# lesliegaga/GPT-SoVITS

Measured on AMD Instinct MI355X. Metric: synthesised audio sec/sec (1/RTF), v2 pipeline, higher is better.
Workload: dtype f16

## Files before the change

### gpt-sovits_amd/csrc/common.h

```cpp
#pragma once
#include <hip/hip_runtime.h>

#include <type_traits>
#include <hip/hip_fp16.h>
#include <stdint.h>
#include <stdio.h>
#include <stdarg.h>
#include <string.h>

#include "../../include/gsv.h"

namespace gsv {

typedef _Float16 h8 __attribute__((ext_vector_type(8)));
typedef _Float16 h4 __attribute__((ext_vector_type(4)));
typedef _Float16 h2 __attribute__((ext_vector_type(2)));
typedef float f4 __attribute__((ext_vector_type(4)));
typedef float f16v __attribute__((ext_vector_type(16)));

void set_error(const char* fmt, ...);

#define GSV_HIP(expr)                                                                   \
  do {                                                                                  \
    hipError_t _e = (expr);                                                             \
// ... 121 lines not shown
  float scale = 1.0f;
  int accumulate = 0;
  int out_f32 = 0;
  int res_f32 = 0;
  int ups_u = 0, ups_pad = 0, ups_cout = 0;
  int Z = 1;
  long long xz = 0, wz = 0, yz = 0, rz = 0;
  unsigned long long* prof = nullptr;
  int bz = 0;
  int xcd_order = 0;
  int w_nt = 0;
  int z_res = 0;
  const int* row_seg = nullptr;
};
enum { ROUTE_GEMM_SK = 1, ROUTE_GEMM_T64 = 2, ROUTE_CONV_WIDE = 3, ROUTE_GEMM_LDS = 4, ROUTE_CONV_LDS = 5, ROUTE_CONV_NARROW = 6,
       ROUTE_CONV_GEMM = 7, ROUTE_CONV_PAIR = 8 };
enum { ROUTE_RES = 1, ROUTE_ACCU = 2, ROUTE_ALLW = 4, ROUTE_WNT = 8, ROUTE_SEG = 16 };
constexpr unsigned long long route_code(int family, int dtype, int p0 = 0, int p1 = 0, int p2 = 0, int p3 = 0, int p4 = 0, int flags = 0) {
  return (unsigned long long)(family & 255) | (unsigned long long)(dtype & 255) << 8 | (unsigned long long)(p0 & 255) << 16 |
         (unsigned long long)(p1 & 255) << 24 | (unsigned long long)(p2 & 255) << 32 | (unsigned long long)(p3 & 255) << 40 |
         (unsigned long long)(p4 & 255) << 48 | (unsigned long long)(flags & 255) << 56;
}
constexpr int route_flags(bool res, bool accu, bool allw = false, bool wnt = false) {
  return (res ? ROUTE_RES : 0) | (accu ? ROUTE_ACCU : 0) | (allw ? ROUTE_ALLW : 0) | (wnt ? ROUTE_WNT : 0);
}
void set_conv_route(unsigned long long code);
int launch_seg_rows(int dtype, int out_f32, void* y, int ldy, int col0, int C, int rows, const int* row_seg, const float* tab, int ldb,
                    hipStream_t s);

int launch_conv_gemm(int dtype, const ConvArgs& a, hipStream_t s);

struct ConvPairArgs {
  const _Float16* x = nullptr;
  const _Float16* w1 = nullptr;
  const float* b1 = nullptr;
  const _Float16* w2 = nullptr;
  const float* b2 = nullptr;
  _Float16* y = nullptr;
  int T = 0, C = 0, taps = 0, dil = 1, ldx = 0, ldy = 0;
  float scale = 1.f;
  int accumulate = 0;
};
bool conv_pair_supported(int dtype, int C, int taps, int dil, int T, bool seg);
bool conv_pair_eligible(int dtype, int C, int taps, int dil, int T, bool seg);
int launch_conv_pair(const ConvPairArgs& a, hipStream_t s);
// ... 27 lines not shown
```

### gpt-sovits_amd/csrc/ops.hip

```cpp
#include "common.h"
#include "engine.h"

namespace gsv {

static thread_local char g_err[1024] = "";
void set_error(const char* fmt, ...) {
  va_list ap;
  va_start(ap, fmt);
  vsnprintf(g_err, sizeof(g_err), fmt, ap);
  va_end(ap);
}
const char* get_error() { return g_err; }

static thread_local unsigned long long g_conv_route = 0;
static thread_local unsigned long long g_pair_route = 0;
void set_conv_route(unsigned long long code) {
  g_conv_route = code;
  if ((code & 255) == ROUTE_CONV_PAIR) g_pair_route = code;
}

template <typename T> __global__ void convert_kernel(const float* __restrict__ s, T* __restrict__ d, long long n) {
  long long i = (long long)blockIdx.x * blockDim.x + threadIdx.x;
  long long stride = (long long)gridDim.x * blockDim.x;
  for (; i < n; i += stride) d[i] = (T)s[i];
// ... 318 lines not shown
  GSV_REQUIRE(word && pos && ids && pos_ids && gamma && beta && y && rows > 0 && n_word > 0 && n_pos > 0, "op_embed_ln: bad argument");
  GSV_REQUIRE(C >= 1 && C <= 1024, "op_embed_ln: C = %d, the row is held in registers up to 1024", C);
  hipLaunchKernelGGL(gsv::embed_ln_kernel, dim3(gsv::cdiv(rows, 4)), dim3(256), 0, (hipStream_t)stream, word, pos, add, ids, pos_ids,
                     gamma, beta, (_Float16*)y, rows, C, n_word, n_pos, eps);
  GSV_HIP(hipGetLastError());
  return GSV_OK;
}

int gsv_op_flash_rel96(const void* qkv, int T, int heads, float scale, const float* rel_k, const float* rel_v, void* vt_scratch,
                       void* out, gsv_stream_t stream) {
  const int H = heads * 96;
  return gsv::launch_flash_rel96_f16(qkv, 3 * H, (const _Float16*)qkv + H, 3 * H, (const _Float16*)qkv + 2 * H, 3 * H, vt_scratch, T, heads,
                                     scale, rel_k, rel_v, out, H, (hipStream_t)stream);
}

int gsv_op_conv1d(const gsv_conv_desc* d, int dtype, gsv_stream_t stream) {
  gsv::ConvArgs a;
  a.x = d->x; a.w = d->w; a.bias = d->bias; a.y = d->y; a.res = d->res; a.gate = d->gate;
  a.T_in = d->T_in; a.T_out = d->T_out; a.Cin = d->Cin; a.Cout = d->Cout; a.taps = d->taps;
  a.stride = d->stride; a.dil = d->dil; a.pad = d->pad;
  a.ldx = d->Cin; a.ldw = d->taps * d->Cin;
  a.pre_act = d->pre_act; a.pre_slope = d->pre_slope; a.post_act = d->post_act; a.scale = d->scale;
  a.accumulate = d->accumulate; a.out_f32 = d->out_f32;
  a.res_f32 = d->res_dtype == 0 ? d->out_f32 : d->res_dtype == 1;
  a.y_col0 = d->y_col0; a.w_nt = d->w_nt; a.z_res = d->z_res;
  if (d->ups_u > 0) {
    a.ups_u = d->ups_u; a.ups_pad = d->ups_pad; a.ups_cout = d->Cout / d->ups_u;
    a.ldy = a.ups_cout; a.ldr = a.ups_cout;
    a.T_virt = d->T_in + d->taps - 1;
  } else {
    a.ldy = d->Cout; a.ldr = d->Cout;
    a.T_virt = d->T_out;
  }
  if (d->ldx > 0) a.ldx = d->ldx;
  if (d->ldw > 0) a.ldw = d->ldw;
  if (d->ldy > 0) { a.ldy = d->ldy; a.ldr = d->ldy; }
  if (d->ldr > 0) a.ldr = d->ldr;
  if (d->Z > 1) { a.Z = d->Z; a.xz = d->xz; a.wz = d->wz; a.yz = d->yz; a.bz = d->bz; a.rz = d->rz ? d->rz : d->yz; }
  return gsv::launch_conv_gemm(dtype, a, (hipStream_t)stream);
}

int gsv_op_frame(const float* x, int n, int frame_len, int hop, int pad, int ld, int T_out, void* out, int dtype, gsv_stream_t stream) {
  GSV_REQUIRE(x && out && n > 0 && frame_len > 0 && hop > 0 && ld >= frame_len && T_out > 0, "op_frame: bad argument");
  GSV_REQUIRE(pad >= 0 && pad < n, "op_frame: reflect padding %d needs more than %d samples", pad, pad);
  GSV_REQUIRE((long long)(T_out - 1) * hop + frame_len - pad <= (long long)n + pad, "op_frame: frames run past the (padded) signal");
  GSV_REQUIRE(dtype == GSV_F16 || dtype == GSV_F32, "op_frame: bad dtype");
  hipStream_t s = (hipStream_t)stream;
  if (dtype == GSV_F16) hipLaunchKernelGGL(gsv::frame_kernel<_Float16>, dim3(T_out), dim3(256), 0, s, x, n, frame_len, hop, pad, ld, T_out, (_Float16*)out);
  else hipLaunchKernelGGL(gsv::frame_kernel<float>, dim3(T_out), dim3(256), 0, s, x, n, frame_len, hop, pad, ld, T_out, (float*)out);
  GSV_HIP(hipGetLastError());
  return GSV_OK;
}

int gsv_op_magnitude(const float* re_im, int T, int bins, float eps, int frame_ld, float* spec, gsv_stream_t stream) {
// ... 104 lines not shown
```

### gpt-sovits_amd/csrc/t2s.hip

```cpp
#include <math.h>
#include <string.h>
#include <stdlib.h>
#include <algorithm>
#include <string>
#include <vector>

#include "t2s_engine.h"

namespace gsv {

typedef float f4v __attribute__((ext_vector_type(4)));


enum { EPI_QKV = 0, EPI_RESID = 1, EPI_RELU = 2, EPI_LOGITS = 3 };

struct DecGemmArgs {
  const float* yin = nullptr;
  const float* gamma = nullptr;
  const float* beta = nullptr;
  float* xres_out = nullptr;
  const void* xin = nullptr;
  const void* w = nullptr;
  const float* bias = nullptr;
  int B = 0, K = 0, N = 0;
// ... 922 lines not shown
                   int32_t* out_tokens, int32_t* out_len, int* steps_run, gsv_stream_t stream) {
  GSV_REQUIRE(h && h->finalized && h->B > 0, "t2s_decode: call gsv_t2s_prefill first");
  struct Clear { gsv_t2s_t* h; ~Clear() { h->row_sampling_next.clear(); } } clear{h};
  GSV_REQUIRE(sp && out_tokens && out_len, "t2s_decode: null argument");
  GSV_REQUIRE(sp->max_steps >= 1, "t2s_decode: max_steps must be >= 1");
  GSV_REQUIRE(noise == nullptr || noise_rows == 1 || noise_rows == h->B, "t2s_decode: noise_rows must be 1 or B");
  return GSV_WITH_T(h, decode<T>(h, sp, noise, noise_rows, out_tokens, out_len, steps_run, (hipStream_t)stream));
}

int gsv_t2s_set_mega(gsv_t2s_t* h, int on) {
  GSV_REQUIRE(h, "t2s_set_mega: null handle");
  h->mega_on = on != 0;
  return GSV_OK;
}

int gsv_t2s_set_debug(gsv_t2s_t* h, const int32_t* force_tokens, float* logits_dump, int32_t* drawn_dump) {
  GSV_REQUIRE(h && h->finalized, "t2s_set_debug: handle not finalized");
  h->dbg_force = force_tokens; h->dbg_dump = logits_dump; h->dbg_drawn = drawn_dump;
  return GSV_OK;
}

int gsv_t2s_debug_stall(gsv_t2s_t* h, int member) {
  GSV_REQUIRE(h && h->finalized && member >= 0 && member < 32, "t2s_debug_stall: bad argument");
  h->dbg_stall = member + 1;
  return GSV_OK;
}

int gsv_t2s_engine_stats(gsv_t2s_t* h, int* engine_available, int* fallbacks, unsigned* last_error3) {
  GSV_REQUIRE(h && h->finalized, "t2s_engine_stats: handle not finalized");
  if (engine_available) *engine_available = h->mega.ready && h->mega.census != 0 ? 1 : 0;
// ... 101 lines not shown
```

### gpt-sovits_amd/csrc/t2s_engine.h

```cpp
#pragma once
#include "engine.h"
#include "t2s_sample.h"
#include "t2s_mega.h"

struct LayerW {
  void *qkv_w = nullptr, *out_w = nullptr, *w1 = nullptr, *w2 = nullptr;
  float *qkv_b = nullptr, *out_b = nullptr, *b1 = nullptr, *b2 = nullptr;
  float *n1w = nullptr, *n1b = nullptr, *n2w = nullptr, *n2b = nullptr;
};

struct gsv_t2s : gsveng::Ctx {
  gsv_t2s() : Ctx("t2s") {}
  gsv_t2s_config cfg;
  int max_batch, max_seq;
  std::vector<LayerW> layers;
  void* bert_w = nullptr; float* bert_b = nullptr;
  float *e_text = nullptr, *e_audio = nullptr, *pe = nullptr;
  void* pred_w = nullptr;
  float alpha_t = 1.f, alpha_a = 1.f;
  int pe_rows = 0;
  void* kv = nullptr; size_t kv_layer_stride = 0;
  int *d_x_len = nullptr, *d_row_off = nullptr, *d_ph_off = nullptr, *d_kv_len = nullptr, *d_active = nullptr,
      *d_step = nullptr, *d_n_active = nullptr, *d_ytok = nullptr;
  int ycap = 0;
// ... 7 lines not shown
  int* h_pinned = nullptr;
  gsv::StepParams* d_sp = nullptr;
  float *ybuf = nullptr, *xres = nullptr, *logits = nullptr;
  void *qbuf = nullptr, *abuf = nullptr, *hbuf = nullptr;
  size_t pf_rows = 0;
  void *pf_x = nullptr, *pf_qkv = nullptr, *pf_attn = nullptr, *pf_h = nullptr;
  void* pf_vt = nullptr; size_t pf_vt_cap = 0;
  float *pf_y = nullptr, *pf_bert = nullptr;
  void* pf_bert_t = nullptr;
  int B = 0, P = 0;
  int max_kv0 = 0;
  gsv::MegaState mega;
  hipEvent_t mega_ev[2] = {nullptr, nullptr};
  float last_decode_ms = 0.f; int last_decode_steps = 0; int last_decode_mode = 0;
  bool mega_on = true;
  const int* dbg_force = nullptr; float* dbg_dump = nullptr; int* dbg_drawn = nullptr; int dbg_stall = 0;
  std::map<int, hipGraphExec_t> graphs;
};

inline void* kv_ptr(gsv_t2s* h, int layer, int which) {
  return (char*)h->kv + ((size_t)(layer * 2 + which) * h->kv_layer_stride) * gsveng::esz(h);
}
```

### gpt-sovits_amd/csrc/t2s_prefill.hip

```cpp
#include <stdlib.h>
#include <type_traits>
#include <vector>

#include "t2s_engine.h"

namespace gsv {

template <typename T>
__global__ void embed_prefill_kernel(const int* __restrict__ phones, const int* __restrict__ prompts,
                                     const int* __restrict__ row_off, const int* __restrict__ ph_off,
                                     const int* __restrict__ x_len, const float* __restrict__ e_text,
                                     const float* __restrict__ e_audio, const float* __restrict__ bertp,
                                     const float* __restrict__ bert_bias, const float* __restrict__ pe, float alpha_t,
                                     float alpha_a, const int* __restrict__ plen, const int* __restrict__ poff, int d,
                                     T* __restrict__ x) {
  const int b = blockIdx.y;
  const int i = blockIdx.x;
  const int X = x_len[b], P = plen[b];
  if (i >= X + P) return;
  T* out = x + (long long)(row_off[b] + i) * d;
  if (i < X) {
    const int id = phones[ph_off[b] + i];
    const float* e = e_text + (long long)id * d;
    const float* bp = bertp ? bertp + (long long)(ph_off[b] + i) * d : nullptr;
// ... 250 lines not shown
  GSV_RC(dalloc(h, (void**)&h->pf_y, rows * d * 4));
  GSV_RC(dalloc(h, (void**)&h->pf_bert, rows * d * 4));
  GSV_RC(dalloc(h, &h->pf_bert_t, rows * (size_t)h->cfg.bert_dim * es));
  h->pf_rows = rows;
  return GSV_OK;
}

ConvArgs linear(const void* x, const void* w, const float* bias, void* y, int rows, int K, int N) {
  ConvArgs g;
  g.x = x; g.w = w; g.bias = bias; g.y = y;
  g.T_in = rows; g.T_out = rows; g.T_virt = rows; g.Cin = K; g.Cout = N; g.ldx = K; g.ldw = K; g.ldy = N;
  return g;
}

bool scalar_prefill_attn() { static const bool v = getenv("GSV_SCALAR_PREFILL_ATTN") != nullptr; return v; }
bool prefill_split_scatter() { static const bool v = getenv("GSV_PREFILL_SPLIT_SCATTER") != nullptr; return v; }

struct PrefillAttnArgs {
  const void* qkv = nullptr;
  void *kc = nullptr, *vc = nullptr, *vt = nullptr, *out = nullptr;
  const int *row_off = nullptr, *x_len = nullptr, *plen = nullptr;
  int B = 0, H = 0, d = 0, smax = 0, maxS = 0;
  bool scalar = false;
  bool split_scatter = false;
};

template <typename T>
int launch_prefill_attention(const PrefillAttnArgs& a, hipStream_t s) {
  const int d = a.d, H = a.H, B = a.B, smax = a.smax, maxS = a.maxS;
  const T* qkv = (const T*)a.qkv;
  T* kc = (T*)a.kc;
// ... 108 lines not shown
  GSV_HIP(hipStreamSynchronize(s));

  const float* bertp = nullptr;
  if (bert) {
    GSV_RC(launch_convert(bert, h->pf_bert_t, h->dtype, (long long)SX * c.bert_dim, s));
    ConvArgs g = linear(h->pf_bert_t, h->bert_w, h->bert_b, h->pf_bert, SX, c.bert_dim, d);
    g.out_f32 = 1;
    GSV_RC(launch_conv_gemm(h->dtype, g, s));
    bertp = h->pf_bert;
  }
  GSV_LAUNCH(embed_prefill_kernel<T>, dim3(maxS, B), dim3(128), 0, s, phones, prompts, h->d_row_off, h->d_ph_off, h->d_x_len,
             h->e_text, h->e_audio, bertp, h->bert_b, h->pe, h->alpha_t, h->alpha_a, d_plen, d_poff, d, (T*)h->pf_x);

  for (int li = 0; li < c.n_layer; ++li) {
    const LayerW& L = h->layers[li];
    GSV_RC(launch_conv_gemm(h->dtype, linear(h->pf_x, L.qkv_w, L.qkv_b, h->pf_qkv, M, d, 3 * d), s));
    GSV_RC(prefill_attention<T>(h, li, maxS, s));
    ConvArgs o = linear(h->pf_attn, L.out_w, L.out_b, h->pf_y, M, d, d);
    o.out_f32 = 1; o.res = h->pf_x; o.ldr = d;
    GSV_RC(launch_conv_gemm(h->dtype, o, s));
    GSV_RC(launch_layernorm(h->dtype, h->pf_y, 1, nullptr, 0, L.n1w, L.n1b, h->pf_x, 0, M, d, 1e-5f, s));
    ConvArgs f1 = linear(h->pf_x, L.w1, L.b1, h->pf_h, M, d, c.ffn_dim);
    f1.post_act = ACT_RELU;
    GSV_RC(launch_conv_gemm(h->dtype, f1, s));
    ConvArgs f2 = linear(h->pf_h, L.w2, L.b2, h->pf_y, M, c.ffn_dim, d);
    f2.out_f32 = 1; f2.res = h->pf_x; f2.ldr = d;
    GSV_RC(launch_conv_gemm(h->dtype, f2, s));
    if (li + 1 < c.n_layer)
      GSV_RC(launch_layernorm(h->dtype, h->pf_y, 1, nullptr, 0, L.n2w, L.n2b, h->pf_x, 0, M, d, 1e-5f, s));
  }
  GSV_LAUNCH(gather_last_kernel, dim3(B), dim3(128), 0, s, h->pf_y, h->d_row_off, h->d_x_len, d_plen, d, h->ybuf);
  return GSV_OK;
}

}

extern "C" {

int gsv_t2s_prefill(gsv_t2s_t* h, const int32_t* phones, const int32_t* phone_lens, int B, const float* bert,
                    const int32_t* prompts, int P, gsv_stream_t stream) {
  GSV_REQUIRE(h && h->finalized, "t2s_prefill: handle not finalized");
  GSV_REQUIRE(phones && phone_lens && (prompts || P == 0), "t2s_prefill: null argument");
// ... 48 lines not shown
```

### gpt-sovits_amd/gsv/AR/models/t2s_model.py

```python
from __future__ import annotations

import ctypes as C
import math
import warnings
from typing import Dict, List, Optional, Sequence

import numpy as np
import torch

from ... import _lib


def _sine_pe(n_pos: int, dim: int) -> torch.Tensor:
    position = torch.arange(0, n_pos, dtype=torch.float32).unsqueeze(1)
    div_term = torch.exp(torch.arange(0, dim, 2, dtype=torch.float32) * -(math.log(10000.0) / dim))
    pe = torch.zeros(n_pos, dim)
    pe[:, 0::2] = torch.sin(position * div_term)
    pe[:, 1::2] = torch.cos(position * div_term)
    return pe


def _host_nonzero(t: torch.Tensor) -> bool:
    try:
        return bool(np.any(t.detach().numpy()))
# ... 125 lines not shown
                                     int(budget), int(seed) & 0xFFFFFFFFFFFFFFFF)
            if early_stop_num not in (-1, None) and budget < int(early_stop_num) + 1:
                sp.early_stop_num = -1
            s = C.c_void_p(self.stream.cuda_stream)
            if ragged:
                plens_h = (C.c_int32 * B)(*plens)
                _lib.check(l.gsv_t2s_prefill_ragged(self._h, phones.data_ptr(), C.cast(lens_h, C.c_void_p), B,
                                                    bert_dev.data_ptr() if bert_dev is not None else None,
                                                    pr.data_ptr(), C.cast(plens_h, C.c_void_p), s),
                           "gsv_t2s_prefill_ragged")
            else:
                _lib.check(l.gsv_t2s_prefill(self._h, phones.data_ptr(), C.cast(lens_h, C.c_void_p), B,
                                             bert_dev.data_ptr() if bert_dev is not None else None,
                                             pr.data_ptr() if P > 0 else None, P, s),
                           "gsv_t2s_prefill")
            if rng_keys is not None:
                seeds_h = (C.c_uint64 * B)(*[int(k[0]) & 0xFFFFFFFFFFFFFFFF for k in rng_keys])
                rows_h = (C.c_int32 * B)(*[int(k[1]) for k in rng_keys])
                _lib.check(l.gsv_t2s_set_row_rng(self._h, C.cast(seeds_h, C.c_void_p), C.cast(rows_h, C.c_void_p), B),
                           "gsv_t2s_set_row_rng")
            if row_sampling is not None:
                rs_h = (_lib.RowSampling * B)(*[_lib.RowSampling(int(k) if k is not None else 0, float(p_ if p_ is not None else 1.0),
                                                                 float(t), float(r)) for k, p_, t, r in row_sampling])
                _lib.check(l.gsv_t2s_set_row_sampling(self._h, rs_h, B), "gsv_t2s_set_row_sampling")
            steps = C.c_int(0)
            dump = None
            if force_tokens is not None or dump_logits:
                ft = None
                if force_tokens is not None:
                    ft = torch.zeros(B, budget, dtype=torch.int32, device=dev)
# ... 87 lines not shown
                                  repetition_penalty: float = 1.35, **kwargs):
        y_list, idx_list = [], []
        for i in range(len(x)):
            y, idx = self.infer_panel_naive(x[i].unsqueeze(0), x_lens[i] if x_lens is not None else None,
                                            prompts[i].unsqueeze(0) if prompts is not None else None,
                                            [bert_feature[i]] if bert_feature[i] is None else bert_feature[i].unsqueeze(0),
                                            top_k, top_p, early_stop_num, temperature,
                                            repetition_penalty, **kwargs)
            y_list.append(y[0])
            idx_list.append(idx)
        return y_list, idx_list

    def set_mega(self, on: bool):
        _lib.check(_lib.lib().gsv_t2s_set_mega(self._h, int(bool(on))), "gsv_t2s_set_mega")

    def debug_stall(self, member: int):
        _lib.check(_lib.lib().gsv_t2s_debug_stall(self._h, int(member)), "gsv_t2s_debug_stall")

    def engine_stats(self):
        av, fb, e3 = C.c_int(0), C.c_int(0), (C.c_uint * 3)()
        _lib.check(_lib.lib().gsv_t2s_engine_stats(self._h, C.byref(av), C.byref(fb), e3), "gsv_t2s_engine_stats")
        return bool(av.value), fb.value, tuple(e3)

    def decode_info(self):
        mode, ms, steps = C.c_int(0), C.c_float(0), C.c_int(0)
        _lib.check(_lib.lib().gsv_t2s_decode_info(self._h, C.byref(mode), C.byref(ms), C.byref(steps)), "gsv_t2s_decode_info")
        return mode.value, ms.value, steps.value

    def debug_logits(self, B: int) -> torch.Tensor:
        out = torch.empty(B, self.vocab_size, dtype=torch.float32, device=self.device)
# ... 15 lines not shown
```

### gpt-sovits_amd/gsv/_lib.py

```python
from __future__ import annotations

import ctypes as C
import os

HERE = os.path.dirname(os.path.abspath(__file__))
LIB_PATH = os.path.join(HERE, "libgsv_hip.so")

GSV_F32, GSV_F16 = 0, 1


class T2SConfig(C.Structure):
    _fields_ = [(n, C.c_int) for n in ("n_layer", "dim", "n_head", "ffn_dim", "vocab", "phoneme_vocab", "bert_dim")]


class SamplingParams(C.Structure):
    _fields_ = [("top_k", C.c_int), ("top_p", C.c_float), ("temperature", C.c_float),
                ("repetition_penalty", C.c_float), ("early_stop_num", C.c_int), ("eos_mask_steps", C.c_int),
                ("max_steps", C.c_int), ("seed", C.c_uint64)]


class RowSampling(C.Structure):
    _fields_ = [("top_k", C.c_int), ("top_p", C.c_float), ("temperature", C.c_float), ("repetition_penalty", C.c_float)]


# ... 43 lines not shown
    "gsv_abi_version": (C.c_int, []),
    "gsv_t2s_create": (C.c_int, [C.POINTER(T2SConfig), C.c_int, C.c_int, C.c_int, C.POINTER(C.c_void_p)]),
    "gsv_t2s_destroy": (None, [C.c_void_p]),
    "gsv_t2s_load_tensor": (C.c_int, [C.c_void_p, C.c_char_p, C.c_void_p, C.c_int64]),
    "gsv_t2s_finalize": (C.c_int, [C.c_void_p]),
    "gsv_t2s_prefill": (C.c_int, [C.c_void_p, C.c_void_p, C.c_void_p, C.c_int, C.c_void_p, C.c_void_p, C.c_int,
                                  C.c_void_p]),
    "gsv_t2s_prefill_ragged": (C.c_int, [C.c_void_p, C.c_void_p, C.c_void_p, C.c_int, C.c_void_p, C.c_void_p,
                                         C.c_void_p, C.c_void_p]),
    "gsv_t2s_set_row_rng": (C.c_int, [C.c_void_p, C.c_void_p, C.c_void_p, C.c_int]),
    "gsv_t2s_set_row_sampling": (C.c_int, [C.c_void_p, C.POINTER(RowSampling), C.c_int]),
    "gsv_t2s_decode": (C.c_int, [C.c_void_p, C.POINTER(SamplingParams), C.c_void_p, C.c_int, C.c_void_p, C.c_void_p,
                                 C.POINTER(C.c_int), C.c_void_p]),
    "gsv_t2s_decode_info": (C.c_int, [C.c_void_p, C.POINTER(C.c_int), C.POINTER(C.c_float), C.POINTER(C.c_int)]),
    "gsv_t2s_set_mega": (C.c_int, [C.c_void_p, C.c_int]),
    "gsv_t2s_engine_stats": (C.c_int, [C.c_void_p, C.POINTER(C.c_int), C.POINTER(C.c_int), C.POINTER(C.c_uint)]),
    "gsv_t2s_set_debug": (C.c_int, [C.c_void_p, C.c_void_p, C.c_void_p, C.c_void_p]),
    "gsv_t2s_debug_stall": (C.c_int, [C.c_void_p, C.c_int]),
    "gsv_t2s_debug_logits": (C.c_int, [C.c_void_p, C.c_void_p, C.c_void_p]),
    "gsv_t2s_time_step": (C.c_int, [C.c_void_p, C.c_int, C.POINTER(C.c_float), C.POINTER(C.c_float), C.c_void_p]),
    "gsv_t2s_debug_set_state": (C.c_int, [C.c_void_p, C.c_int, C.c_int]),
    "gsv_t2s_step_bytes": (C.c_int64, [C.c_void_p, C.POINTER(C.c_int64)]),
    "gsv_vits_create": (C.c_int, [C.POINTER(VitsConfig), C.c_int, C.POINTER(C.c_void_p)]),
    "gsv_vits_destroy": (None, [C.c_void_p]),
    "gsv_vits_load_tensor": (C.c_int, [C.c_void_p, C.c_char_p, C.c_void_p, C.c_int64]),
    "gsv_vits_finalize": (C.c_int, [C.c_void_p]),
    "gsv_vits_set_refer": (C.c_int, [C.c_void_p, C.POINTER(C.c_void_p), C.POINTER(C.c_int), C.c_int, C.c_int,
                                     C.c_void_p]),
    "gsv_vits_set_refer_sv": (C.c_int, [C.c_void_p, C.POINTER(C.c_void_p), C.POINTER(C.c_int), C.c_int, C.POINTER(C.c_void_p),
                                        C.c_int, C.c_void_p]),
# ... 54 lines not shown
    "gsv_bwe_load_tensor": (C.c_int, [C.c_void_p, C.c_char_p, C.c_void_p, C.c_int64]),
    "gsv_bwe_finalize": (C.c_int, [C.c_void_p]),
    "gsv_bwe_out_len": (C.c_int, [C.c_void_p, C.c_int, C.c_int]),
    "gsv_bwe_forward": (C.c_int, [C.c_void_p, C.c_void_p, C.c_int, C.c_int, C.c_int, C.c_void_p, C.c_void_p]),
    "gsv_bwe_debug_tensor": (C.c_int, [C.c_void_p, C.c_char_p, C.c_void_p, C.c_int64, C.POINTER(C.c_int64), C.c_void_p]),
    "gsv_aa_act_forward": (C.c_int, [C.c_void_p, C.c_void_p, C.c_void_p, C.c_void_p, C.c_void_p, C.c_void_p,
                                     C.c_int, C.c_int, C.c_int, C.c_int, C.c_void_p]),
    "gsv_op_flash_attn64": (C.c_int, [C.c_void_p, C.c_int, C.c_int, C.c_float, C.c_void_p, C.c_void_p, C.c_void_p]),
    "gsv_op_flash_attn64_seg": (C.c_int, [C.c_void_p, C.c_int, C.POINTER(C.c_int32), C.c_int, C.c_float, C.c_void_p, C.c_void_p,
                                          C.c_void_p]),
    "gsv_op_embed_ln": (C.c_int, [C.c_void_p, C.c_int, C.c_void_p, C.c_int, C.c_void_p, C.c_void_p, C.c_void_p, C.c_void_p, C.c_void_p,
                                  C.c_void_p, C.c_int, C.c_int, C.c_float, C.c_void_p]),
    "gsv_op_flash_rel96": (C.c_int, [C.c_void_p, C.c_int, C.c_int, C.c_float, C.c_void_p, C.c_void_p, C.c_void_p, C.c_void_p,
                                     C.c_void_p]),
    "gsv_op_conv1d": (C.c_int, [C.POINTER(ConvDesc), C.c_int, C.c_void_p]),
    "gsv_debug_last_conv_route": (C.c_uint64, [C.c_int]),
    "gsv_debug_last_pair_route": (C.c_uint64, [C.c_int]),
    "gsv_op_frame": (C.c_int, [C.c_void_p, C.c_int, C.c_int, C.c_int, C.c_int, C.c_int, C.c_int, C.c_void_p, C.c_int, C.c_void_p]),
    "gsv_op_magnitude": (C.c_int, [C.c_void_p, C.c_int, C.c_int, C.c_float, C.c_int, C.c_void_p, C.c_void_p]),
    "gsv_op_conv_pair": (C.c_int, [C.c_void_p, C.c_void_p, C.c_void_p, C.c_void_p, C.c_void_p, C.c_void_p, C.c_int, C.c_int, C.c_int,
                                  C.c_int, C.c_float, C.c_int, C.c_void_p]),
    "gsv_op_conv_pair_seg": (C.c_int, [C.c_void_p, C.c_void_p, C.c_void_p, C.c_void_p, C.c_void_p, C.c_void_p, C.c_int, C.c_int, C.c_int,
                                      C.c_int, C.c_float, C.c_int, C.c_void_p, C.c_void_p]),
    "gsv_op_aa_act_cl": (C.c_int, [C.c_void_p, C.c_void_p, C.c_int, C.c_int, C.c_void_p, C.c_void_p, C.c_int, C.c_void_p, C.c_void_p,
                                  C.c_void_p, C.c_int, C.c_int, C.c_void_p]),
    "gsv_op_aff_mix": (C.c_int, [C.c_void_p, C.c_void_p, C.c_void_p, C.c_longlong, C.c_void_p, C.c_void_p]),
    "gsv_op_time_mean": (C.c_int, [C.c_void_p, C.c_int, C.c_int, C.c_void_p, C.c_void_p]),
    "gsv_op_channel_norm": (C.c_int, [C.c_void_p, C.c_int, C.c_int, C.c_void_p, C.c_void_p, C.c_float, C.c_int, C.c_void_p,
                                      C.c_void_p, C.c_int, C.c_void_p]),
    "gsv_op_channel_norm_seg": (C.c_int, [C.c_void_p, C.c_int, C.c_int, C.c_int, C.POINTER(C.c_int32), C.POINTER(C.c_int32), C.c_void_p,
# ... 76 lines not shown
```

### include/gsv.h

```cpp
#ifndef GSV_H_
#define GSV_H_

#include <stdint.h>

#ifdef __cplusplus
extern "C" {
#endif

#define GSV_OK 0
#define GSV_ERR_ARG (-1)
#define GSV_ERR_HIP (-2)
#define GSV_ERR_STATE (-3)

#define GSV_F32 0
#define GSV_F16 1

typedef void* gsv_stream_t;

int gsv_init(int device);
const char* gsv_last_error(void);
int gsv_abi_version(void);

typedef struct gsv_t2s gsv_t2s_t;

// ... 31 lines not shown

typedef struct {
  int top_k;
  float top_p;
  float temperature;
  float repetition_penalty;
} gsv_row_sampling_t;

int gsv_t2s_set_row_sampling(gsv_t2s_t* h, const gsv_row_sampling_t* rows, int B);

int gsv_t2s_decode(gsv_t2s_t* h, const gsv_sampling_params* sp, const float* noise, int noise_rows,
                   int32_t* out_tokens, int32_t* out_len, int* steps_run, gsv_stream_t stream);

int gsv_t2s_decode_info(gsv_t2s_t* h, int* mode, float* device_ms, int* steps);
int gsv_t2s_set_mega(gsv_t2s_t* h, int on);
int gsv_t2s_engine_stats(gsv_t2s_t* h, int* engine_available, int* fallbacks, unsigned* last_error3);
int gsv_t2s_set_debug(gsv_t2s_t* h, const int32_t* force_tokens, float* logits_dump, int32_t* drawn_dump);
int gsv_t2s_debug_stall(gsv_t2s_t* h, int member);
int gsv_t2s_debug_logits(gsv_t2s_t* h, float* out, gsv_stream_t stream);
int gsv_t2s_time_step(gsv_t2s_t* h, int iters, float* step_ms, float* attn_ms, gsv_stream_t stream);
int gsv_t2s_debug_set_state(gsv_t2s_t* h, int B, int kv_len);
int64_t gsv_t2s_step_bytes(gsv_t2s_t* h, int64_t* attn_bytes);

typedef struct gsv_vits gsv_vits_t;

typedef struct {
  int inter_channels, hidden_channels, filter_channels, n_heads, n_layers, kernel_size;
  int gin_channels, n_symbols, ssl_dim, n_bins, upsample_initial_channel;
  int n_ups;
  int up_rates[8];
  int up_kernels[8];
  int n_resblocks;
  int rb_kernels[4];
  int rb_dilations[4][3];
// ... 130 lines not shown
  int z_res;
} gsv_conv_desc;
int gsv_op_flash_attn64(const void* qkv, int T, int heads, float scale, void* vt_scratch, void* out, gsv_stream_t stream);
int gsv_op_flash_attn64_seg(const void* qkv, int n_seg, const int32_t* seg_lens, int heads, float scale, void* vt_scratch, void* out,
                            gsv_stream_t stream);
int gsv_op_embed_ln(const float* word, int n_word, const float* pos, int n_pos, const float* add, const int32_t* ids,
                    const int32_t* pos_ids, const float* gamma, const float* beta, void* y, int rows, int C, float eps,
                    gsv_stream_t stream);
int gsv_op_flash_rel96(const void* qkv, int T, int heads, float scale, const float* rel_k, const float* rel_v, void* vt_scratch,
                       void* out, gsv_stream_t stream);
int gsv_op_decode_attn(const void* q, const void* kc, const void* vc, const int32_t* kv_len, const int32_t* active, int B, int H,
                       int smax, int dtype, void* out, gsv_stream_t stream);
int gsv_op_prefill_attn(const void* qkv, const int32_t* x_len, const int32_t* p_len, int B, int H, int d, int smax, int dtype,
                        int route, void* kc, void* vc, void* out, gsv_stream_t stream);
int gsv_op_conv1d(const gsv_conv_desc* d, int dtype, gsv_stream_t stream);
uint64_t gsv_debug_last_conv_route(int reset);
uint64_t gsv_debug_last_pair_route(int reset);
int gsv_op_layernorm(const void* x, const void* res, const float* gamma, const float* beta, void* y, int rows,
                     int C, float eps, int dtype, gsv_stream_t stream);
int gsv_op_lora_delta(const void* x, void* y, int Tn, int DB, int K, int N, int n_proj, const int* slots, int n_slots,
                      const void* const* blocks, const int* rp, const float* gate, int dtype, gsv_stream_t stream);
int gsv_op_frame(const float* x, int n, int frame_len, int hop, int pad, int ld, int T_out, void* out, int dtype, gsv_stream_t stream);
int gsv_op_magnitude(const float* re_im, int T, int bins, float eps, int frame_ld, float* spec, gsv_stream_t stream);
int gsv_op_conv_pair(const void* x, const void* w1, const float* b1, const void* w2, const float* b2, void* y, int T, int C, int taps,
                     int dil, float scale, int accumulate, gsv_stream_t stream);
int gsv_op_conv_pair_seg(const void* x, const void* w1, const float* b1, const void* w2, const float* b2, void* y, int T, int C, int taps,
                         int dil, float scale, int accumulate, const int32_t* row_seg, gsv_stream_t stream);
int gsv_op_aa_act_cl(const void* x, void* y, int T, int C, const float* alpha, const float* beta, int logscale,
                     const int32_t* row_seg, const int32_t* seg_start, const int32_t* seg_len, int n_seg, int dtype,
                     gsv_stream_t stream);
// ... 25 lines not shown
```

Measured before the change: 2858.

## Add LDS-pipelined panel GEMM kernel for large T2S prefill linears

Adds a new f16 MFMA GEMM kernel that streams activation and weight panels into a multi-stage LDS ring with direct global-to-LDS loads, and fuses bias, residual and ReLU into an LDS-staged epilogue. Tile shape is chosen by a wave-quantisation cost model. The T2S prefill routes its QKV, output and FFN linears through it when the row count is large enough and the tile count suits it (default mode 2), and otherwise keeps the existing dispatcher. The aim is better data reuse and overlap on long prefills, at the cost of a new code path that only fires for large prompts and adds debug and selection APIs.

```diff
diff --git a/gpt-sovits_amd/csrc/common.h b/gpt-sovits_amd/csrc/common.h
--- a/gpt-sovits_amd/csrc/common.h
+++ b/gpt-sovits_amd/csrc/common.h
@@ -159,7 +159,7 @@
   const int* row_seg = nullptr;
 };
 enum { ROUTE_GEMM_SK = 1, ROUTE_GEMM_T64 = 2, ROUTE_CONV_WIDE = 3, ROUTE_GEMM_LDS = 4, ROUTE_CONV_LDS = 5, ROUTE_CONV_NARROW = 6,
-       ROUTE_CONV_GEMM = 7, ROUTE_CONV_PAIR = 8 };
+       ROUTE_CONV_GEMM = 7, ROUTE_CONV_PAIR = 8, ROUTE_GEMM_PANEL = 9 };
 enum { ROUTE_RES = 1, ROUTE_ACCU = 2, ROUTE_ALLW = 4, ROUTE_WNT = 8, ROUTE_SEG = 16 };
 constexpr unsigned long long route_code(int family, int dtype, int p0 = 0, int p1 = 0, int p2 = 0, int p3 = 0, int p4 = 0, int flags = 0) {
   return (unsigned long long)(family & 255) | (unsigned long long)(dtype & 255) << 8 | (unsigned long long)(p0 & 255) << 16 |
@@ -174,6 +174,10 @@
                     hipStream_t s);
 
 int launch_conv_gemm(int dtype, const ConvArgs& a, hipStream_t s);
+bool gemm_panel_eligible(int dtype, const ConvArgs& a);
+int gemm_panel_auto_tile(const ConvArgs& a, int* wgs_out);
+int launch_gemm_panel(int dtype, const ConvArgs& a, int tile, hipStream_t s);
+int launch_gemm_panel_as_dispatcher(int dtype, const ConvArgs& a, hipStream_t s);
 
 struct ConvPairArgs {
   const _Float16* x = nullptr;
diff --git a/gpt-sovits_amd/csrc/gemm_panel.hip b/gpt-sovits_amd/csrc/gemm_panel.hip
--- /dev/null
+++ b/gpt-sovits_amd/csrc/gemm_panel.hip
@@ -0,0 +1,274 @@
+#include "conv_launch.h"
+#include "mfma_frag.h"
+
+namespace gsv {
+
+namespace {
+
+struct PanelArgs {
+  const _Float16* x; const _Float16* w; const float* bias; void* y; const _Float16* res;
+  int M, N, K, ldx, ldw, ldy, ldr;
+  float scale;
+  int relu, xcd_order, gy;
+};
+
+typedef __attribute__((address_space(3))) unsigned char lds_byte;
+
+__device__ __forceinline__ void glds16(const void* gsrc, unsigned lds_dst) {
+  unsigned keep;
+  asm volatile("s_mov_b32 %0, m0\n\ts_mov_b32 m0, %2\n\ts_nop 0\n\tglobal_load_lds_dwordx4 %1, off\n\ts_mov_b32 m0, %0"
+               : "=&s"(keep) : "v"(gsrc), "s"(lds_dst) : "memory");
+}
+template <int N> __device__ __forceinline__ void wait_dma_barrier() {
+  asm volatile("s_waitcnt vmcnt(%0)\n\ts_waitcnt lgkmcnt(0)\n\ts_barrier" ::"i"(N) : "memory");
+}
+
+template <int TB, int CB, int WT, int WN, int NS, bool RES, bool SUM2 = false>
+__global__ __launch_bounds__(WT * WN * 64) void gemm_panel_kernel(PanelArgs a) {
+  constexpr int NW = WT * WN, NT = NW * 64;
+  constexpr int TR = TB * 32, TC = CB * 32, RT = TR + TC;
+  constexpr int TM = CB / WN, TN = TB / WT;
+  constexpr int L = RT / 8 / NW;
+  constexpr int STAGE = RT * 128;
+  static_assert(CB % WN == 0 && TB % WT == 0 && (RT / 8) % NW == 0 && TR % 8 == 0, "tile / wave geometry");
+  static_assert(L * (NS - 2) <= 63, "vmcnt is a 6-bit count");
+  extern __shared__ __attribute__((aligned(16))) unsigned char smem[];
+  const int tid = threadIdx.x, lane = tid & 63;
+  const int wave = __builtin_amdgcn_readfirstlane(tid >> 6);
+  const int r = lane & 31, h = lane >> 5;
+  const int wt = wave / WN, wn = wave % WN;
+  int bx, by;
+  {
+    const int n = gridDim.x;
+    const int vid = a.xcd_order ? xcd_virtual_id(blockIdx.x, n) : (int)blockIdx.x;
+    by = vid % a.gy; bx = vid / a.gy;
+  }
+  const int t0 = bx * TR, cout0 = by * TC;
+  const int K = a.K;
+  const unsigned lds0 = (unsigned)(uintptr_t)(lds_byte*)smem;
+
+  const _Float16* src[L];
+#pragma unroll
+  for (int i = 0; i < L; ++i) {
+    const int row = (i * NW + wave) * 8 + (lane >> 3);
+    const int slot = (lane & 7) ^ ((row >> 1) & 7);
+    if (row < TR) src[i] = a.x + (long long)min(t0 + row, a.M - 1) * a.ldx + slot * 8;
+    else src[i] = a.w + (long long)min(cout0 + row - TR, a.N - 1) * a.ldw + slot * 8;
+  }
+  auto issue = [&](int c, int buf) {
+#pragma unroll
+    for (int i = 0; i < L; ++i) glds16(src[i] + c * 64, lds0 + buf * STAGE + (i * NW + wave) * 1024);
+  };
+
+  const int nch = K / 64;
+  issue(0, 0);
+
+  constexpr int VW = RES ? 4 : 8;
+  constexpr int LDO = TC + 4, PR = TN * 32, IPR = TC / VW, NI = PR * IPR / NT;
+  static_assert(NT % IPR == 0 && (PR * IPR) % NT == 0, "epilogue geometry");
+  static_assert(PR * LDO * 4 <= NS * STAGE, "the epilogue tile lives in the ring");
+  const int ecg = tid % IPR, ec = cout0 + VW * ecg;
+  const bool col_ok = ec < a.N;
+  const int ecl = min(ec, a.N - VW);
+  float ebias[VW];
+#pragma unroll
+  for (int j = 0; j < VW; ++j) ebias[j] = a.bias[ecl + j];
+  h4 rv[RES ? WT * NI : 1];
+  if (RES) {
+#pragma unroll
+    for (int q = 0; q < WT * NI; ++q) {
+      const int pass = q / NI, e = q - pass * NI;
+      const int t = min(t0 + pass * PR + (tid + e * NT) / IPR, a.M - 1);
+      rv[q] = *(const h4*)(a.res + (long long)t * a.ldr + ecl);
+    }
+  }
+#pragma unroll
+  for (int i = 1; i <= NS - 2; ++i)
+    if (i < nch) issue(i, i);
+
+  constexpr int NA = SUM2 ? 2 : 1;
+  f16v acc[NA][TM][TN];
+#pragma unroll
+  for (int p = 0; p < NA; ++p)
+#pragma unroll
+    for (int m = 0; m < TM; ++m)
+#pragma unroll
+      for (int n = 0; n < TN; ++n)
+#pragma unroll
+        for (int i = 0; i < 16; ++i) acc[p][m][n][i] = 0.f;
+
+  const int sw = (r >> 1) & 7;
+  int buf = 0, nbuf = NS - 1;
+  for (int c = 0; c < nch; ++c) {
+    if (c + NS - 2 < nch) wait_dma_barrier<L * (NS - 2)>();
+    else wait_dma_barrier<0>();
+    if (c + NS - 1 < nch) issue(c + NS - 1, nbuf);
+    const unsigned char* xb = smem + buf * STAGE;
+    const unsigned char* wb = xb + TR * 128;
+    h8 af[2][TM], bf[2][TN];
+    auto frags = [&](int ks, int set) {
+      const int off = ((2 * ks + h) ^ sw) * 16;
+#pragma unroll
+      for (int m = 0; m < TM; ++m) af[set][m] = *(const h8*)(wb + ((wn * TM + m) * 32 + r) * 128 + off);
+#pragma unroll
+      for (int n = 0; n < TN; ++n) bf[set][n] = *(const h8*)(xb + ((wt * TN + n) * 32 + r) * 128 + off);
+    };
+    frags(0, 0);
+#pragma unroll
+    for (int ks = 0; ks < 4; ++ks) {
+      if (ks < 3) frags(ks + 1, (ks + 1) & 1);
+#pragma unroll
+      for (int m = 0; m < TM; ++m)
+#pragma unroll
+        for (int n = 0; n < TN; ++n) mma32l(acc[SUM2 ? (ks & 1) : 0][m][n], af[ks & 1][m], bf[ks & 1][n]);
+    }
+    buf = buf + 1 == NS ? 0 : buf + 1;
+    nbuf = nbuf + 1 == NS ? 0 : nbuf + 1;
+  }
+
+#pragma unroll
+  for (int j = 0; j < VW; ++j) asm volatile("" : "+v"(ebias[j]));
+  if (RES) {
+#pragma unroll
+    for (int q = 0; q < WT * NI; ++q) asm volatile("" : "+v"(rv[q]));
+  }
+  float* os = (float*)smem;
+#pragma unroll
+  for (int pass = 0; pass < WT; ++pass) {
+    lds_barrier();
+    if (wt == pass) {
+#pragma unroll
+      for (int m = 0; m < TM; ++m)
+#pragma unroll
+        for (int n = 0; n < TN; ++n) {
+          const int tl = n * 32 + r;
+#pragma unroll
+          for (int g = 0; g < 4; ++g) {
+            const int cl = (wn * TM + m) * 32 + 8 * g + 4 * h;
+            f4 v4;
+#pragma unroll
+            for (int i = 0; i < 4; ++i) v4[i] = SUM2 ? acc[0][m][n][4 * g + i] + acc[NA - 1][m][n][4 * g + i] : acc[0][m][n][4 * g + i];
+            *(f4*)(os + tl * LDO + cl) = v4;
+          }
+        }
+    }
+    lds_barrier();
+    auto items = [&](auto relu_tag) {
+#pragma unroll
+      for (int e = 0; e < NI; ++e) {
+        const int tl = (tid + e * NT) / IPR;
+        const int t = t0 + pass * PR + tl;
+        if (!(t < a.M && col_ok)) continue;
+        float v[VW];
+#pragma unroll
+        for (int j4 = 0; j4 < VW / 4; ++j4) {
+          const f4 av = *(const f4*)(os + tl * LDO + VW * ecg + 4 * j4);
+#pragma unroll
+          for (int j = 0; j < 4; ++j) {
+            float u = av[j] + ebias[4 * j4 + j];
+            if (RES) u += (float)rv[RES ? pass * NI + e : 0][j];
+            u *= a.scale;
+            if (decltype(relu_tag)::value) u = fmaxf(u, 0.f);
+            v[4 * j4 + j] = u;
+          }
+        }
+        const long long yoff = (long long)t * a.ldy + ec;
+        if constexpr (RES) {
+          *(f4*)((float*)a.y + yoff) = (f4){v[0], v[1], v[2], v[3]};
+        } else {
+          h8 o;
+#pragma unroll
+          for (int j = 0; j < 8; ++j) o[j] = (_Float16)v[j];
+          *(h8*)((_Float16*)a.y + yoff) = o;
+        }
+      }
+    };
+    if (!RES && a.relu) items(std::true_type{});
+    else items(std::false_type{});
+  }
+}
+
+template <int TB, int CB, int WT, int WN, int NS, bool SUM2 = false> int launch_tile(const PanelArgs& a0, bool res, hipStream_t s) {
+  PanelArgs a = a0;
+  const int gx = cdiv(a.M, TB * 32);
+  a.gy = cdiv(a.N, CB * 32);
+  const dim3 grid(gx * a.gy), block(WT * WN * 64);
+  const size_t lds = (size_t)NS * (TB + CB) * 32 * 128;
+  static_assert((size_t)NS * (TB + CB) * 32 * 128 <= LDS_CAP, "LDS budget");
+  if (res)
+    return launch_routed<gemm_panel_kernel<TB, CB, WT, WN, NS, true, SUM2>, LDS_CAP>(
+        route_code(ROUTE_GEMM_PANEL, GSV_F16, TB, CB, SUM2 ? 1 : 0, 0, 0, route_flags(true, false)), grid, block, lds, s, a);
+  return launch_routed<gemm_panel_kernel<TB, CB, WT, WN, NS, false, SUM2>, LDS_CAP>(
+      route_code(ROUTE_GEMM_PANEL, GSV_F16, TB, CB, SUM2 ? 1 : 0, 0, 0, route_flags(false, false)), grid, block, lds, s, a);
+}
+
+}
+
+bool gemm_panel_eligible(int dtype, const ConvArgs& a) {
+  if (dtype != GSV_F16) return false;
+  if (!a.x || !a.w || !a.y || !a.bias) return false;
+  if (a.taps != 1 || a.stride != 1 || a.pad != 0 || a.ups_u > 0 || a.Z > 1 || a.row_seg) return false;
+  if (a.gate || a.accumulate || a.pre_act != ACT_NONE || a.y_col0 != 0) return false;
+  if (a.T_in < 1 || a.T_out != a.T_in || a.T_virt != a.T_in) return false;
+  if (a.Cin < 64 || a.Cin % 64 != 0 || a.Cout < 8 || a.Cout % 8 != 0) return false;
+  if (!operands_aligned<8>(a) || a.ldx < a.Cin || a.ldw < a.Cin || a.ldy < a.Cout) return false;
+  if ((uintptr_t)a.y % 16 != 0) return false;
+  if (a.res) {
+    if (!a.out_f32 || a.res_f32 || a.post_act != ACT_NONE) return false;
+    if (a.ldy % 4 != 0 || a.ldr % 4 != 0 || a.ldr < a.Cout || (uintptr_t)a.res % 8 != 0) return false;
+  } else {
+    if (a.out_f32 || (a.post_act != ACT_NONE && a.post_act != ACT_RELU)) return false;
+    if (a.ldy % 8 != 0) return false;
+  }
+  return true;
+}
+
+int gemm_panel_auto_tile(const ConvArgs& a, int* wgs_out) {
+  static const int rows[3] = {192, 192, 96}, cols[3] = {256, 192, 128};
+  long long wgs[3];
+  int best = -1;
+  long long best_cost = 0;
+  for (int i = 0; i < 3; ++i) {
+    wgs[i] = (long long)cdiv(a.T_in, rows[i]) * cdiv(a.Cout, cols[i]);
+    const long long cost = (wgs[i] + 255) / 256 * rows[i] * cols[i];
+    if (best < 0 || cost < best_cost) { best = i; best_cost = cost; }
+  }
+  if (wgs[best] > 256)
+    for (int i = 0; i < best; ++i)
+      if (wgs[i] >= 256) { best = i; break; }
+  if (wgs_out) *wgs_out = (int)std::min<long long>(wgs[best], 1 << 30);
+  return best + 1;
+}
+
+int gemm_panel_dispatcher_sum(const ConvArgs& a) {
+  const ConvSwitches& sw = conv_switches();
+  const long long tiles128 = (long long)cdiv(a.T_virt, 128) * cdiv(a.Cout, 128);
+  if (!sw.no_gemm_sk && a.Cin >= 256 && a.Cout >= 64 && tiles128 < sw.sk_max_tiles && a.T_virt <= 2048)
+    return sw.gemm_t64 && a.Cin % 512 == 0 ? 1 : -1;
+  if (!sw.no_conv_lds && a.T_virt >= 512 && a.Cout >= 96) return 0;
+  return -1;
+}
+
+int launch_gemm_panel(int dtype, const ConvArgs& c, int tile, hipStream_t s) {
+  if (!gemm_panel_eligible(dtype, c) || tile < 0 || tile > 4) return 1;
+  PanelArgs a;
+  a.x = (const _Float16*)c.x; a.w = (const _Float16*)c.w; a.bias = c.bias; a.y = c.y; a.res = (const _Float16*)c.res;
+  a.M = c.T_in; a.N = c.Cout; a.K = c.Cin; a.ldx = c.ldx; a.ldw = c.ldw; a.ldy = c.ldy; a.ldr = c.ldr;
+  a.scale = c.scale; a.relu = c.post_act == ACT_RELU;
+  a.xcd_order = conv_switches().gemm_xcd ? 1 : 0;
+  a.gy = 0;
+  if (tile == 0) tile = gemm_panel_auto_tile(c, nullptr);
+  if (tile == 1) return launch_tile<6, 8, 2, 4, 2>(a, c.res != nullptr, s);
+  if (tile == 2) return launch_tile<6, 6, 2, 3, 3>(a, c.res != nullptr, s);
+  if (tile == 4) return launch_tile<3, 4, 1, 4, 5, true>(a, c.res != nullptr, s);
+  return launch_tile<3, 4, 1, 4, 5>(a, c.res != nullptr, s);
+}
+
+int launch_gemm_panel_as_dispatcher(int dtype, const ConvArgs& c, hipStream_t s) {
+  if (!gemm_panel_eligible(dtype, c)) return 1;
+  const int sum = gemm_panel_dispatcher_sum(c);
+  if (sum < 0) return 1;
+  return launch_gemm_panel(dtype, c, sum == 1 ? 4 : 0, s);
+}
+
+}
diff --git a/gpt-sovits_amd/csrc/ops.hip b/gpt-sovits_amd/csrc/ops.hip
--- a/gpt-sovits_amd/csrc/ops.hip
+++ b/gpt-sovits_amd/csrc/ops.hip
@@ -356,7 +356,7 @@
                                      scale, rel_k, rel_v, out, H, (hipStream_t)stream);
 }
 
-int gsv_op_conv1d(const gsv_conv_desc* d, int dtype, gsv_stream_t stream) {
+static gsv::ConvArgs conv_desc_args(const gsv_conv_desc* d) {
   gsv::ConvArgs a;
   a.x = d->x; a.w = d->w; a.bias = d->bias; a.y = d->y; a.res = d->res; a.gate = d->gate;
   a.T_in = d->T_in; a.T_out = d->T_out; a.Cin = d->Cin; a.Cout = d->Cout; a.taps = d->taps;
@@ -379,7 +379,21 @@
   if (d->ldy > 0) { a.ldy = d->ldy; a.ldr = d->ldy; }
   if (d->ldr > 0) a.ldr = d->ldr;
   if (d->Z > 1) { a.Z = d->Z; a.xz = d->xz; a.wz = d->wz; a.yz = d->yz; a.bz = d->bz; a.rz = d->rz ? d->rz : d->yz; }
-  return gsv::launch_conv_gemm(dtype, a, (hipStream_t)stream);
+  return a;
+}
+
+int gsv_op_conv1d(const gsv_conv_desc* d, int dtype, gsv_stream_t stream) {
+  return gsv::launch_conv_gemm(dtype, conv_desc_args(d), (hipStream_t)stream);
+}
+
+int gsv_op_gemm_panel(const gsv_conv_desc* d, int dtype, int tile, gsv_stream_t stream) {
+  GSV_REQUIRE(d, "op_gemm_panel: null descriptor");
+  GSV_REQUIRE(tile >= 0 && tile <= 4, "op_gemm_panel: tile %d is not a member of the family (0 = by shape, 1..4)", tile);
+  const gsv::ConvArgs a = conv_desc_args(d);
+  GSV_REQUIRE(gsv::gemm_panel_eligible(dtype, a), "op_gemm_panel: the descriptor is not one of the prefill's three GEMM forms");
+  const int rc = gsv::launch_gemm_panel(dtype, a, tile, (hipStream_t)stream);
+  GSV_REQUIRE(rc != 1, "op_gemm_panel: not eligible");
+  return rc;
 }
 
 int gsv_op_frame(const float* x, int n, int frame_len, int hop, int pad, int ld, int T_out, void* out, int dtype, gsv_stream_t stream) {
diff --git a/gpt-sovits_amd/csrc/t2s.hip b/gpt-sovits_amd/csrc/t2s.hip
--- a/gpt-sovits_amd/csrc/t2s.hip
+++ b/gpt-sovits_amd/csrc/t2s.hip
@@ -960,6 +960,24 @@
   return GSV_OK;
 }
 
+int gsv_t2s_debug_kv(gsv_t2s_t* h, int layer, int which, int row, int n_pos, void* out) {
+  GSV_REQUIRE(h && h->finalized && out, "t2s_debug_kv: null argument or handle not finalized");
+  GSV_REQUIRE(layer >= 0 && layer < h->cfg.n_layer && (which == 0 || which == 1) && row >= 0 && row < h->max_batch && n_pos >= 1 &&
+                  n_pos <= h->max_seq, "t2s_debug_kv: layer %d / which %d / row %d / n_pos %d outside the arena", layer, which, row, n_pos);
+  const size_t es = esz(h), H = h->cfg.n_head, pitch = (size_t)h->max_seq * 32 * es;
+  GSV_HIP(hipDeviceSynchronize());
+  GSV_HIP(hipMemcpy2D(out, (size_t)n_pos * 32 * es, (const char*)kv_ptr(h, layer, which) + (size_t)row * H * pitch, pitch,
+                      (size_t)n_pos * 32 * es, H, hipMemcpyDeviceToHost));
+  return GSV_OK;
+}
+
+int gsv_t2s_set_prefill_gemm(gsv_t2s_t* h, int mode) {
+  GSV_REQUIRE(h, "t2s_set_prefill_gemm: null handle");
+  GSV_REQUIRE(mode >= 0 && mode <= 2, "t2s_set_prefill_gemm: mode %d (0 dispatcher, 1 panel, 2 panel from the threshold)", mode);
+  h->prefill_gemm = mode;
+  return GSV_OK;
+}
+
 int gsv_t2s_set_debug(gsv_t2s_t* h, const int32_t* force_tokens, float* logits_dump, int32_t* drawn_dump) {
   GSV_REQUIRE(h && h->finalized, "t2s_set_debug: handle not finalized");
   h->dbg_force = force_tokens; h->dbg_dump = logits_dump; h->dbg_drawn = drawn_dump;
diff --git a/gpt-sovits_amd/csrc/t2s_engine.h b/gpt-sovits_amd/csrc/t2s_engine.h
--- a/gpt-sovits_amd/csrc/t2s_engine.h
+++ b/gpt-sovits_amd/csrc/t2s_engine.h
@@ -45,6 +45,7 @@
   hipEvent_t mega_ev[2] = {nullptr, nullptr};
   float last_decode_ms = 0.f; int last_decode_steps = 0; int last_decode_mode = 0;
   bool mega_on = true;
+  int prefill_gemm = 2;
   const int* dbg_force = nullptr; float* dbg_dump = nullptr; int* dbg_drawn = nullptr; int dbg_stall = 0;
   std::map<int, hipGraphExec_t> graphs;
 };
diff --git a/gpt-sovits_amd/csrc/t2s_prefill.hip b/gpt-sovits_amd/csrc/t2s_prefill.hip
--- a/gpt-sovits_amd/csrc/t2s_prefill.hip
+++ b/gpt-sovits_amd/csrc/t2s_prefill.hip
@@ -288,7 +288,25 @@
 }
 
 bool scalar_prefill_attn() { static const bool v = getenv("GSV_SCALAR_PREFILL_ATTN") != nullptr; return v; }
+bool no_prefill_panel() { static const bool v = getenv("GSV_NO_PREFILL_PANEL") != nullptr; return v; }
 bool prefill_split_scatter() { static const bool v = getenv("GSV_PREFILL_SPLIT_SCATTER") != nullptr; return v; }
+
+constexpr int PANEL_MIN_ROWS = 2049;
+bool panel_pays(const ConvArgs& g) {
+  if (g.T_in < PANEL_MIN_ROWS) return false;
+  int wgs = 0;
+  gemm_panel_auto_tile(g, &wgs);
+  const long long tiles128 = (long long)((g.T_in + 127) / 128) * ((g.Cout + 127) / 128);
+  return !(tiles128 <= 256 && wgs > 256);
+}
+int prefill_gemm(gsv_t2s* h, const ConvArgs& g, hipStream_t s) {
+  const int mode = no_prefill_panel() ? 0 : h->prefill_gemm;
+  if (mode == 1 || (mode == 2 && panel_pays(g))) {
+    const int rc = launch_gemm_panel_as_dispatcher(h->dtype, g, s);
+    if (rc != 1) return rc;
+  }
+  return launch_conv_gemm(h->dtype, g, s);
+}
 
 struct PrefillAttnArgs {
   const void* qkv = nullptr;
@@ -427,18 +445,18 @@
 
   for (int li = 0; li < c.n_layer; ++li) {
     const LayerW& L = h->layers[li];
-    GSV_RC(launch_conv_gemm(h->dtype, linear(h->pf_x, L.qkv_w, L.qkv_b, h->pf_qkv, M, d, 3 * d), s));
+    GSV_RC(prefill_gemm(h, linear(h->pf_x, L.qkv_w, L.qkv_b, h->pf_qkv, M, d, 3 * d), s));
     GSV_RC(prefill_attention<T>(h, li, maxS, s));
     ConvArgs o = linear(h->pf_attn, L.out_w, L.out_b, h->pf_y, M, d, d);
     o.out_f32 = 1; o.res = h->pf_x; o.ldr = d;
-    GSV_RC(launch_conv_gemm(h->dtype, o, s));
+    GSV_RC(prefill_gemm(h, o, s));
     GSV_RC(launch_layernorm(h->dtype, h->pf_y, 1, nullptr, 0, L.n1w, L.n1b, h->pf_x, 0, M, d, 1e-5f, s));
     ConvArgs f1 = linear(h->pf_x, L.w1, L.b1, h->pf_h, M, d, c.ffn_dim);
     f1.post_act = ACT_RELU;
-    GSV_RC(launch_conv_gemm(h->dtype, f1, s));
+    GSV_RC(prefill_gemm(h, f1, s));
     ConvArgs f2 = linear(h->pf_h, L.w2, L.b2, h->pf_y, M, c.ffn_dim, d);
     f2.out_f32 = 1; f2.res = h->pf_x; f2.ldr = d;
-    GSV_RC(launch_conv_gemm(h->dtype, f2, s));
+    GSV_RC(prefill_gemm(h, f2, s));
     if (li + 1 < c.n_layer)
       GSV_RC(launch_layernorm(h->dtype, h->pf_y, 1, nullptr, 0, L.n2w, L.n2b, h->pf_x, 0, M, d, 1e-5f, s));
   }
diff --git a/gpt-sovits_amd/gsv/AR/models/t2s_model.py b/gpt-sovits_amd/gsv/AR/models/t2s_model.py
--- a/gpt-sovits_amd/gsv/AR/models/t2s_model.py
+++ b/gpt-sovits_amd/gsv/AR/models/t2s_model.py
@@ -163,6 +163,7 @@
                                              bert_dev.data_ptr() if bert_dev is not None else None,
                                              pr.data_ptr() if P > 0 else None, P, s),
                            "gsv_t2s_prefill")
+            self.last_prefill_route = int(l.gsv_debug_last_conv_route(0))
             if rng_keys is not None:
                 seeds_h = (C.c_uint64 * B)(*[int(k[0]) & 0xFFFFFFFFFFFFFFFF for k in rng_keys])
                 rows_h = (C.c_int32 * B)(*[int(k[1]) for k in rng_keys])
@@ -280,6 +281,14 @@
     def set_mega(self, on: bool):
         _lib.check(_lib.lib().gsv_t2s_set_mega(self._h, int(bool(on))), "gsv_t2s_set_mega")
 
+    def set_prefill_gemm(self, mode: int):
+        _lib.check(_lib.lib().gsv_t2s_set_prefill_gemm(self._h, int(mode)), "gsv_t2s_set_prefill_gemm")
+
+    def debug_kv(self, layer: int, which: int, row: int, n_pos: int):
+        out = torch.empty(self.num_head, n_pos, 32, dtype=self.dtype)
+        _lib.check(_lib.lib().gsv_t2s_debug_kv(self._h, layer, which, row, n_pos, out.data_ptr()), "gsv_t2s_debug_kv")
+        return out
+
     def debug_stall(self, member: int):
         _lib.check(_lib.lib().gsv_t2s_debug_stall(self._h, int(member)), "gsv_t2s_debug_stall")
 
diff --git a/gpt-sovits_amd/gsv/_lib.py b/gpt-sovits_amd/gsv/_lib.py
--- a/gpt-sovits_amd/gsv/_lib.py
+++ b/gpt-sovits_amd/gsv/_lib.py
@@ -81,6 +81,8 @@
                                  C.POINTER(C.c_int), C.c_void_p]),
     "gsv_t2s_decode_info": (C.c_int, [C.c_void_p, C.POINTER(C.c_int), C.POINTER(C.c_float), C.POINTER(C.c_int)]),
     "gsv_t2s_set_mega": (C.c_int, [C.c_void_p, C.c_int]),
+    "gsv_t2s_set_prefill_gemm": (C.c_int, [C.c_void_p, C.c_int]),
+    "gsv_t2s_debug_kv": (C.c_int, [C.c_void_p, C.c_int, C.c_int, C.c_int, C.c_int, C.c_void_p]),
     "gsv_t2s_engine_stats": (C.c_int, [C.c_void_p, C.POINTER(C.c_int), C.POINTER(C.c_int), C.POINTER(C.c_uint)]),
     "gsv_t2s_set_debug": (C.c_int, [C.c_void_p, C.c_void_p, C.c_void_p, C.c_void_p]),
     "gsv_t2s_debug_stall": (C.c_int, [C.c_void_p, C.c_int]),
@@ -165,6 +167,7 @@
     "gsv_op_flash_rel96": (C.c_int, [C.c_void_p, C.c_int, C.c_int, C.c_float, C.c_void_p, C.c_void_p, C.c_void_p, C.c_void_p,
                                      C.c_void_p]),
     "gsv_op_conv1d": (C.c_int, [C.POINTER(ConvDesc), C.c_int, C.c_void_p]),
+    "gsv_op_gemm_panel": (C.c_int, [C.POINTER(ConvDesc), C.c_int, C.c_int, C.c_void_p]),
     "gsv_debug_last_conv_route": (C.c_uint64, [C.c_int]),
     "gsv_debug_last_pair_route": (C.c_uint64, [C.c_int]),
     "gsv_op_frame": (C.c_int, [C.c_void_p, C.c_int, C.c_int, C.c_int, C.c_int, C.c_int, C.c_int, C.c_void_p, C.c_int, C.c_void_p]),
diff --git a/include/gsv.h b/include/gsv.h
--- a/include/gsv.h
+++ b/include/gsv.h
@@ -69,10 +69,12 @@
 
 int gsv_t2s_decode_info(gsv_t2s_t* h, int* mode, float* device_ms, int* steps);
 int gsv_t2s_set_mega(gsv_t2s_t* h, int on);
+int gsv_t2s_set_prefill_gemm(gsv_t2s_t* h, int mode);
 int gsv_t2s_engine_stats(gsv_t2s_t* h, int* engine_available, int* fallbacks, unsigned* last_error3);
 int gsv_t2s_set_debug(gsv_t2s_t* h, const int32_t* force_tokens, float* logits_dump, int32_t* drawn_dump);
 int gsv_t2s_debug_stall(gsv_t2s_t* h, int member);
 int gsv_t2s_debug_logits(gsv_t2s_t* h, float* out, gsv_stream_t stream);
+int gsv_t2s_debug_kv(gsv_t2s_t* h, int layer, int which, int row, int n_pos, void* out);
 int gsv_t2s_time_step(gsv_t2s_t* h, int iters, float* step_ms, float* attn_ms, gsv_stream_t stream);
 int gsv_t2s_debug_set_state(gsv_t2s_t* h, int B, int kv_len);
 int64_t gsv_t2s_step_bytes(gsv_t2s_t* h, int64_t* attn_bytes);
@@ -233,6 +235,7 @@
 int gsv_op_prefill_attn(const void* qkv, const int32_t* x_len, const int32_t* p_len, int B, int H, int d, int smax, int dtype,
                         int route, void* kc, void* vc, void* out, gsv_stream_t stream);
 int gsv_op_conv1d(const gsv_conv_desc* d, int dtype, gsv_stream_t stream);
+int gsv_op_gemm_panel(const gsv_conv_desc* d, int dtype, int tile, gsv_stream_t stream);
 uint64_t gsv_debug_last_conv_route(int reset);
 uint64_t gsv_debug_last_pair_route(int reset);
 int gsv_op_layernorm(const void* x, const void* res, const float* gamma, const float* beta, void* y, int rows,
```

New measurement: 2904, median of 6. 1.02x the previous value.
